# Lzcstan/DrugLAMP

Measured on AMD Instinct MI355X. Metric: drug-protein pairs/sec training step, higher is better.
Workload: dtype bf16; 1 GPU; DrugLAMP training step (cls step, epoch 1; fwd+bwd+grad all-reduce+AdamW), BindingDB-shaped synthetic pairs (512 drug nodes/tokens, 2304 protein tokens = 256 sites, pre-extracted 384-d/640-d LLM embeddings), global batch 256 = 256 per GPU x 1; per_gpu_batch=256, global_batch=256, parallelism=dp1, step_kind=cls, epoch=1, hip_graph=False, protein_seq_len=2304, distinct_batches=8, first_touch_steps=8, padding_rows=computed once, protein_cnn_rows=distinct rows, streams=independent branches on side HIP streams

## Files before the change

druglamp_amd/csrc/attention.hip:

```cpp
#include "tiles.cuh"

namespace {
using namespace dltile;

struct AttnP {
  const char *Q, *K, *V, *O, *dO;
  char *Out, *dQ, *dK, *dV;
  float *LSE, *Delta, *raw;
  int64_t q_ps, q_hs, q_rs, k_ps, k_hs, k_rs, v_ps, v_hs, v_rs, o_ps, o_hs, o_rs, o_ss;
  int64_t do_ps, do_hs, do_rs, do_ss, dq_ps, dq_hs, dq_rs, dk_ps, dk_hs, dk_rs, dv_ps, dv_hs, dv_rs;
  int P, H, S, shift, Lq, Lk;
  float scale;
  int algo;
  int tail_start;
  float tail_bias;
};

template <int QT, int NKT>
__device__ __forceinline__ void add_tail_bias_t(f32x4 (&s)[QT][NKT], int k0, int g, int tail_start, float tb) {
#pragma unroll
  for (int kt = 0; kt < NKT; ++kt)
#pragma unroll
    for (int r = 0; r < 4; ++r)
      if (k0 + kt * 16 + 4 * g + r >= tail_start) {
// ... 685 lines not shown
        sdo.store(dOs);
        if (threadIdx.x < QSB) {
          const int q = q0 + threadIdx.x;
          lse_s[threadIdx.x] = q < p.Lq ? p.LSE[statbase + q] * LOG2E : INFINITY;
          del_s[threadIdx.x] = q < p.Lq ? p.Delta[statbase + q] : 0.f;
        }
        __syncthreads();
        if (qb + 1 < nqb) {
          sq.load(Qb, p.q_rs, q0 + QSB, p.Lq);
          sdo.load(dOb, p.do_rs, q0 + QSB, p.Lq);
        }
      }
      const char* Qt = RES ? Qs + q0 * TL::RB : Qs;
      const char* dOt = RES ? dOs + q0 * TL::RB : dOs;
      const float* lse_t = RES ? lse_s + q0 : lse_s;
      const float* del_t = RES ? del_s + q0 : del_s;
      f32x4 s[KT][NQT], dp[KT][NQT];
#pragma unroll
      for (int qt = 0; qt < NQT; ++qt) {
#pragma unroll
        for (int kt = 0; kt < KT; ++kt) { s[kt][qt] = f32x4{0.f, 0.f, 0.f, 0.f}; dp[kt][qt] = f32x4{0.f, 0.f, 0.f, 0.f}; }
#pragma unroll
        for (int kf = 0; kf < NKF; ++kf) {
          const u32x4 qa = frag_kc<T, HD>(Qt, qt * 16, kf, il, g);
          const u32x4 da = frag_kc<T, HD>(dOt, qt * 16, kf, il, g);
#pragma unroll
          for (int kt = 0; kt < KT; ++kt) {
            s[kt][qt] = Mma<T>::mma(qa, kfr[kt][kf], s[kt][qt]);
            dp[kt][qt] = Mma<T>::mma(da, vfr[kt][kf], dp[kt][qt]);
          }
        }
        const f32x4 l4 = *reinterpret_cast<const f32x4*>(lse_t + qt * 16 + 4 * g);
        const f32x4 d4 = *reinterpret_cast<const f32x4*>(del_t + qt * 16 + 4 * g);
        if (has_tail) {
#pragma unroll
          for (int kt = 0; kt < KT; ++kt) s[kt][qt] += kbl[kt];
        }
#pragma unroll
        for (int kt = 0; kt < KT; ++kt)
#pragma unroll
          for (int r = 0; r < 4; ++r) {
            const float pv = fast_exp2(s[kt][qt][r] * c - l4[r]);
            s[kt][qt][r] = pv;
            dp[kt][qt][r] = pv * (dp[kt][qt][r] - d4[r]);
          }
      }
#pragma unroll
      for (int qp = 0; qp < NQP; ++qp) {
        u32x4 pb[KT], sb[KT];
#pragma unroll
        for (int kt = 0; kt < KT; ++kt) {
          pb[kt] = frag_from_acc<T>(&s[kt][qp * CT]);
          sb[kt] = frag_from_acc<T>(&dp[kt][qp * CT]);
        }
#pragma unroll
        for (int d = 0; d < NDT; ++d) {
          const u32x4 dota = frag_tr<T, HD>(dOt, qp * KF, d * 16, il, g);
          const u32x4 qta = frag_tr<T, HD>(Qt, qp * KF, d * 16, il, g);
#pragma unroll
          for (int kt = 0; kt < KT; ++kt) {
            dv[d][kt] = Mma<T>::mma(dota, pb[kt], dv[d][kt]);
            dk[d][kt] = Mma<T>::mma(qta, sb[kt], dk[d][kt]);
          }
        }
      }
      if constexpr (!RES) __syncthreads();
    }
  }
  T* dKb = reinterpret_cast<T*>(p.dK) + (int64_t)pa * p.dk_ps + (int64_t)h * p.dk_hs;
  T* dVb = reinterpret_cast<T*>(p.dV) + (int64_t)pa * p.dv_ps + (int64_t)h * p.dv_hs;
#pragma unroll
  for (int kt = 0; kt < KT; ++kt) {
    const int key = kw0 + kt * 16 + il;
    if (key < p.Lk) {
#pragma unroll
      for (int d = 0; d < NDT; ++d) {
        store4_fam<4, T>(dKb + (int64_t)key * p.dk_rs + d * 16 + 4 * g, dk[d][kt] * p.scale);
        store4_fam<4, T>(dVb + (int64_t)key * p.dv_rs + d * 16 + 4 * g, dv[d][kt]);
      }
    }
  }
}

template <typename T, int HD, int KT, bool TAILK = false>
__global__ __launch_bounds__(ATT_THREADS, 1) void attn_bwd_dkv_ring_kernel(const AttnP p) {
  using TL = ATile<T, HD>;
  constexpr int KF = Mma<T>::KF, NKF = HD / KF, NDT = HD / 16, CT = KF / 16;
  constexpr int QSB = 64, NQP = QSB / KF;
  constexpr int KVB = 4 * KT * 16;
  constexpr int TILE = QSB * TL::RB, STAGE = 2 * TILE;
  constexpr int NCH = QSB * TL::CPR / ATT_THREADS;
  static_assert(sizeof(T) == 2 && QSB * TL::CPR % ATT_THREADS == 0, "bf16 tiles, whole DMA instructions");
  __shared__ __attribute__((aligned(16))) char smem[2 * STAGE + 2 * 2 * QSB * sizeof(float)];
  const uint32_t smem_lds = (uint32_t)(size_t)(__attribute__((address_space(3))) char*)smem;
  float* stat_s = reinterpret_cast<float*>(smem + 2 * STAGE);
  const int tid = threadIdx.x, lane = tid & 63, wave = tid >> 6, il = lane & 15, g = lane >> 4;
  const int kb = blockIdx.x, h = blockIdx.y, pa = blockIdx.z;
  const T* Kb = reinterpret_cast<const T*>(p.K) + (int64_t)pa * p.k_ps + (int64_t)h * p.k_hs;
  const T* Vb = reinterpret_cast<const T*>(p.V) + (int64_t)pa * p.v_ps + (int64_t)h * p.v_hs;
  const int kw0 = kb * KVB + wave * KT * 16;
  const float c = p.scale * LOG2E;

  u32x4 kfr[KT][NKF], vfr[KT][NKF];
#pragma unroll
  for (int kt = 0; kt < KT; ++kt) {
    const int key = kw0 + kt * 16 + il;
    const bool ok = key < p.Lk;
#pragma unroll
    for (int kf = 0; kf < NKF; ++kf) {
      kfr[kt][kf] = frag_global<T>(Kb + (int64_t)key * p.k_rs, ok, kf, g);
      vfr[kt][kf] = frag_global<T>(Vb + (int64_t)key * p.v_rs, ok, kf, g);
    }
  }
  f32x4 dk[NDT][KT], dv[NDT][KT];
#pragma unroll
  for (int d = 0; d < NDT; ++d)
#pragma unroll
    for (int kt = 0; kt < KT; ++kt) { dk[d][kt] = f32x4{0.f, 0.f, 0.f, 0.f}; dv[d][kt] = f32x4{0.f, 0.f, 0.f, 0.f}; }
  const bool has_tail = TAILK && kw0 + KT * 16 > p.tail_start;
  float kbl[KT];
#pragma unroll
  for (int kt = 0; kt < KT; ++kt) kbl[kt] = (TAILK && kw0 + kt * 16 + il >= p.tail_start) ? p.tail_bias : 0.f;

  const int nqb = (p.Lq + QSB - 1) / QSB;
  for (int seg = 0; seg < p.S; ++seg) {
    const int qprob = seg == 0 ? pa : (pa + p.shift) % p.P;
    const T* Qb = reinterpret_cast<const T*>(p.Q) + (int64_t)qprob * p.q_ps + (int64_t)h * p.q_hs;
    const T* dOb = reinterpret_cast<const T*>(p.dO) + (int64_t)seg * p.do_ss + (int64_t)pa * p.do_ps + (int64_t)h * p.do_hs;
    const int64_t statbase = (((int64_t)seg * p.P + pa) * p.H + h) * p.Lq;
    auto issue = [&](int qb, int buf) {
      const char* zero = reinterpret_cast<const char*>(zero_page);
      const uint32_t sb = smem_lds + (uint32_t)buf * STAGE;
#pragma unroll
      for (int i = 0; i < NCH; ++i) {
        const int cc = tid + i * ATT_THREADS;
        const int row = cc / TL::CPR, ch = (cc % TL::CPR) ^ TL::swz(row);
        const int q = qb * QSB + row;
        const char* qs_ = q < p.Lq ? reinterpret_cast<const char*>(Qb + (int64_t)q * p.q_rs + ch * TL::EPC) : zero;
        const char* ds_ = q < p.Lq ? reinterpret_cast<const char*>(dOb + (int64_t)q * p.do_rs + ch * TL::EPC) : zero;
        const uint32_t off = __builtin_amdgcn_readfirstlane((uint32_t)((wave * 64 + i * ATT_THREADS) * 16));
        att_dma16(qs_, sb + off);
        att_dma16(ds_, sb + TILE + off);
      }
      if (tid < QSB) {
        const int q = qb * QSB + tid;
        stat_s[(buf * 2 + 0) * QSB + tid] = q < p.Lq ? p.LSE[statbase + q] * LOG2E : INFINITY;
        stat_s[(buf * 2 + 1) * QSB + tid] = q < p.Lq ? p.Delta[statbase + q] : 0.f;
      }
    };
    if (seg > 0) att_barrier();
    issue(0, 0);
    for (int qb = 0; qb < nqb; ++qb) {
      att_wait_all();
      att_barrier();
      if (qb + 1 < nqb) issue(qb + 1, (qb + 1) & 1);
      const char* Qt = smem + (qb & 1) * STAGE;
      const char* dOt = Qt + TILE;
      const float* lse_t = stat_s + ((qb & 1) * 2 + 0) * QSB;
      const float* del_t = stat_s + ((qb & 1) * 2 + 1) * QSB;
#pragma unroll
      for (int qp = 0; qp < NQP; ++qp) {
        f32x4 s[KT][CT], dp[KT][CT];
#pragma unroll
        for (int ci = 0; ci < CT; ++ci) {
          const int qt = qp * CT + ci;
#pragma unroll
          for (int kt = 0; kt < KT; ++kt) { s[kt][ci] = f32x4{0.f, 0.f, 0.f, 0.f}; dp[kt][ci] = f32x4{0.f, 0.f, 0.f, 0.f}; }
#pragma unroll
          for (int kf = 0; kf < NKF; ++kf) {
            const u32x4 qa = frag_kc<T, HD>(Qt, qt * 16, kf, il, g);
            const u32x4 da = frag_kc<T, HD>(dOt, qt * 16, kf, il, g);
#pragma unroll
            for (int kt = 0; kt < KT; ++kt) {
              s[kt][ci] = Mma<T>::mma(qa, kfr[kt][kf], s[kt][ci]);
              dp[kt][ci] = Mma<T>::mma(da, vfr[kt][kf], dp[kt][ci]);
            }
          }
          const f32x4 l4 = *reinterpret_cast<const f32x4*>(lse_t + qt * 16 + 4 * g);
          const f32x4 d4 = *reinterpret_cast<const f32x4*>(del_t + qt * 16 + 4 * g);
          if (has_tail) {
#pragma unroll
            for (int kt = 0; kt < KT; ++kt) s[kt][ci] += kbl[kt];
          }
#pragma unroll
          for (int kt = 0; kt < KT; ++kt)
#pragma unroll
            for (int r = 0; r < 4; ++r) {
              const float pv = fast_exp2(s[kt][ci][r] * c - l4[r]);
              s[kt][ci][r] = pv;
              dp[kt][ci][r] = pv * (dp[kt][ci][r] - d4[r]);
            }
        }
        u32x4 pb[KT], sb[KT];
#pragma unroll
        for (int kt = 0; kt < KT; ++kt) {
          pb[kt] = frag_from_acc<T>(&s[kt][0]);
          sb[kt] = frag_from_acc<T>(&dp[kt][0]);
        }
#pragma unroll
        for (int d = 0; d < NDT; ++d) {
          const u32x4 dota = frag_tr<T, HD>(dOt, qp * KF, d * 16, il, g);
          const u32x4 qta = frag_tr<T, HD>(Qt, qp * KF, d * 16, il, g);
#pragma unroll
          for (int kt = 0; kt < KT; ++kt) {
            dv[d][kt] = Mma<T>::mma(dota, pb[kt], dv[d][kt]);
            dk[d][kt] = Mma<T>::mma(qta, sb[kt], dk[d][kt]);
          }
        }
      }
    }
  }
  T* dKb = reinterpret_cast<T*>(p.dK) + (int64_t)pa * p.dk_ps + (int64_t)h * p.dk_hs;
  T* dVb = reinterpret_cast<T*>(p.dV) + (int64_t)pa * p.dv_ps + (int64_t)h * p.dv_hs;
#pragma unroll
  for (int kt = 0; kt < KT; ++kt) {
    const int key = kw0 + kt * 16 + il;
    if (key < p.Lk) {
#pragma unroll
      for (int d = 0; d < NDT; ++d) {
        store4_fam<4, T>(dKb + (int64_t)key * p.dk_rs + d * 16 + 4 * g, dk[d][kt] * p.scale);
        store4_fam<4, T>(dVb + (int64_t)key * p.dv_rs + d * 16 + 4 * g, dv[d][kt]);
      }
    }
  }
}

__device__ __forceinline__ int ds_swz(int key) { return (((key >> 2) & 1) << 1) | ((key >> 3) & 1); }
template <typename T, int HD>
__global__ __launch_bounds__(512, 1) void attn_bwd_fused_kernel(const AttnP p) {
  static_assert(sizeof(T) == 2 && HD == 64, "bf16, head_dim 64");
  using TL = ATile<T, HD>;
  constexpr int KF = Mma<T>::KF, NKF = HD / KF, NDT = HD / 16, KT = 2, NQT = 2, QBLK = 32, NT = 512, NST = 4;
  constexpr int TILE = QBLK * TL::RB;
  constexpr int STAGE = 3 * TILE;
  constexpr int IMG = 256 * TL::RB;
  constexpr int DSB = 256 * 64;
  __shared__ __attribute__((aligned(16))) char smem[NST * STAGE + 2 * IMG + 2 * DSB + NST * (64 + QBLK) * (int)sizeof(float)];
  char* ring = smem;
  char* Ks = smem + NST * STAGE;
  char* Vs = Ks + IMG;
  char* dSs = Vs + IMG;
  float* lse_s = reinterpret_cast<float*>(dSs + 2 * DSB);
  float* del_s = lse_s + NST * 64;
  const int tid = threadIdx.x, lane = tid & 63, il = lane & 15, g = lane >> 4;
  const int wave = __builtin_amdgcn_readfirstlane(tid >> 6);
  const int h = blockIdx.y;
  const int a0 = blockIdx.z;
  const int npass = p.S == 2 ? 4 : 1;
  const int kw0 = wave * KT * 16;
  const int qt_o = wave & 1, dt_o = wave >> 1;
  const float c = p.scale * LOG2E;
  const int nblk = (p.Lq + QBLK - 1) / QBLK;
  const int G = npass * nblk;
  const uint32_t smem_base = (uint32_t)(size_t)(__attribute__((address_space(3))) char*)smem;
  const char* zero = reinterpret_cast<const char*>(zero_page);

  const int nd = wave <= 4 ? 2 : 1;
  int pf_pass = 0, pf_blk = 0, pf_stage = 0;
  const T* pfA = nullptr;
  const T* pfO = nullptr;
  const float* pfL = nullptr;
  int64_t pfA_rs = 0;
  auto pf_setup = [&]() {
    const int pa = pf_pass < 2 ? a0 : a0 + p.shift;
    const int seg = pf_pass & 1;
    const int qprob = seg == 0 ? pa : (pa + p.shift) % p.P;
    if (wave < 4) { pfA = reinterpret_cast<const T*>(p.Q) + ((int64_t)qprob * p.q_ps + (int64_t)h * p.q_hs); pfA_rs = p.q_rs; }
    else { pfA = reinterpret_cast<const T*>(p.dO) + ((int64_t)seg * p.do_ss + (int64_t)pa * p.do_ps + (int64_t)h * p.do_hs); pfA_rs = p.do_rs; }
    pfO = reinterpret_cast<const T*>(p.O) + ((int64_t)seg * p.o_ss + (int64_t)pa * p.o_ps + (int64_t)h * p.o_hs);
    pfL = p.LSE + (((int64_t)seg * p.P + pa) * p.H + h) * p.Lq;
  };
  pf_setup();
  auto issue_next = [&]() {
    const uint32_t st = smem_base + (uint32_t)(pf_stage * STAGE);
    const int row = 8 * (wave & 3) + (lane >> 3), q = pf_blk * QBLK + row;
    const int ch = (lane & 7) ^ TL::swz(row);
    const bool ok = q < p.Lq;
    lds_dma16(ok ? reinterpret_cast<const char*>(pfA + (int64_t)q * pfA_rs + ch * TL::EPC) : zero,
              st + (uint32_t)((wave < 4 ? 0 : TILE) + (wave & 3) * 1024));
    if (wave < 4) {
      lds_dma16(ok ? reinterpret_cast<const char*>(pfO + (int64_t)q * p.o_rs + ch * TL::EPC) : zero, st + (uint32_t)(2 * TILE + wave * 1024));
    } else if (wave == 4) {
      const int ql = pf_blk * QBLK + (lane & 31);
      lds_dma4(pfL + (ql < p.Lq ? ql : p.Lq - 1), smem_base + (uint32_t)((char*)lse_s - smem) + (uint32_t)(pf_stage * 256));
    }
    pf_stage = (pf_stage + 1) & (NST - 1);
    if (++pf_blk == nblk) {
      pf_blk = 0;
      if (++pf_pass < npass) pf_setup();
    }
  };
  auto issue_kv = [&](int pa) {
    const T* Kb = reinterpret_cast<const T*>(p.K) + (int64_t)pa * p.k_ps + (int64_t)h * p.k_hs;
    const T* Vb = reinterpret_cast<const T*>(p.V) + (int64_t)pa * p.v_ps + (int64_t)h * p.v_hs;
#pragma unroll
    for (int i = 0; i < 4; ++i) {
      const int row = (i * 8 + wave) * 8 + (lane >> 3);
      const int ch = (lane & 7) ^ TL::swz(row);
      const bool ok = row < p.Lk;
      lds_dma16(ok ? reinterpret_cast<const char*>(Kb + (int64_t)row * p.k_rs + ch * TL::EPC) : zero,
                smem_base + (uint32_t)(Ks - smem) + (uint32_t)((i * 8 + wave) * 1024));
      lds_dma16(ok ? reinterpret_cast<const char*>(Vb + (int64_t)row * p.v_rs + ch * TL::EPC) : zero,
                smem_base + (uint32_t)(Vs - smem) + (uint32_t)((i * 8 + wave) * 1024));
    }
  };
// ... 69 lines not shown
            dp[kt] = Mma<T>::mma(da, vfr[kt][kf], dp[kt]);
          }
        }
        const f32x4 l4 = *reinterpret_cast<const f32x4*>(lse_t + qt * 16 + 4 * g) * LOG2E;
        const f32x4 d4 = *reinterpret_cast<const f32x4*>(del_t + qt * 16 + 4 * g);
#pragma unroll
        for (int kt = 0; kt < KT; ++kt) {
#pragma unroll
          for (int r = 0; r < 4; ++r) {
            const float pv = fast_exp2(s[kt][r] * c - l4[r]);
            s[kt][r] = pv;
            dp[kt][r] = pv * (dp[kt][r] - d4[r]);
          }
          pb[kt][2 * qt] = pack_bf16x2(s[kt][0], s[kt][1]);
          pb[kt][2 * qt + 1] = pack_bf16x2(s[kt][2], s[kt][3]);
          sb[kt][2 * qt] = pack_bf16x2(dp[kt][0], dp[kt][1]);
          sb[kt][2 * qt + 1] = pack_bf16x2(dp[kt][2], dp[kt][3]);
        }
      }
#pragma unroll
      for (int kt = 0; kt < KT; ++kt) {
        const int key = kw0 + kt * 16 + il, sw = ds_swz(key);
        *reinterpret_cast<u32x2*>(dSb + key * 64 + (((0 + (g >> 1)) ^ sw) << 4) + 8 * (g & 1)) = u32x2{sb[kt][0], sb[kt][1]};
        *reinterpret_cast<u32x2*>(dSb + key * 64 + (((2 + (g >> 1)) ^ sw) << 4) + 8 * (g & 1)) = u32x2{sb[kt][2], sb[kt][3]};
      }
#pragma unroll
      for (int d = 0; d < NDT; ++d) {
        const u32x4 dota = frag_tr<T, HD>(dOt, 0, d * 16, il, g);
        const u32x4 qta = frag_tr<T, HD>(Qt, 0, d * 16, il, g);
#pragma unroll
        for (int kt = 0; kt < KT; ++kt) {
          dv[d][kt] = Mma<T>::mma(dota, pb[kt], dv[d][kt]);
          dk[d][kt] = Mma<T>::mma(qta, sb[kt], dk[d][kt]);
        }
      }
      if (gb + 3 < G) {
        if (nd == 2) vm_wait<2>(); else vm_wait<1>();
      } else {
        vm_wait<0>();
      }
      __syncthreads();
      if (gb + 2 < G) form_delta((gb + 2) & (NST - 1));
      f32x4 dq = {0.f, 0.f, 0.f, 0.f};
#pragma unroll
      for (int cki = 0; cki < 8; ++cki) {
        const int r0 = cki * 32 + 4 * g + (il >> 2), sw = ds_swz(r0);
        const uint32_t off = (uint32_t)(r0 * 64 + (((2 * qt_o + ((il & 3) >> 1)) ^ sw) << 4) + (il & 1) * 8);
        const u32x2 lo = lds_read_tr16(dSb, off);
        const u32x2 hi = lds_read_tr16(dSb, off + 16 * 64);
        dq = Mma<T>::mma(ktr[cki], u32x4{lo[0], lo[1], hi[0], hi[1]}, dq);
      }
      if (add_share) asm volatile("s_waitcnt vmcnt(0)" : "+v"(prevw) :: "memory");
      if (qo < p.Lq) {
        f32x4 v = dq * p.scale;
        if (add_share) {
          v = v + f32x4{bf16lo(prevw[0]), bf16hi(prevw[0]), bf16lo(prevw[1]), bf16hi(prevw[1])};
          store4_fam<4, T>(dst, v);
        } else if (npass == 1) {
          store4_fam<4, T>(dst, v);
        } else {
          store4<T>(dst, v);
        }
      }
    }
    if (!new_kv || npass == 1) {
      T* dKb = reinterpret_cast<T*>(p.dK) + (int64_t)pa * p.dk_ps + (int64_t)h * p.dk_hs;
      T* dVb = reinterpret_cast<T*>(p.dV) + (int64_t)pa * p.dv_ps + (int64_t)h * p.dv_hs;
#pragma unroll
      for (int kt = 0; kt < KT; ++kt) {
        const int key = kw0 + kt * 16 + il;
        if (key < p.Lk) {
#pragma unroll
          for (int d = 0; d < NDT; ++d) {
            store4_fam<4, T>(dKb + (int64_t)key * p.dk_rs + d * 16 + 4 * g, dk[d][kt] * p.scale);
            store4_fam<4, T>(dVb + (int64_t)key * p.dv_rs + d * 16 + 4 * g, dv[d][kt]);
          }
        }
      }
    }
  }
}

template <typename T> constexpr int fwd_qt() { return sizeof(T) == 2 ? 2 : 1; }

int check_common(const char* who, int dtype, int head_dim, int nseg, int P, int H, int Lq, int Lk,
                 const int64_t* strides, int nstrides) {
  DL_CHECK_ARG(dtype == DL_F32 || dtype == DL_BF16, DL_ERR_ARG, "%s: bad dtype", who);
  DL_CHECK_ARG(head_dim == 64 || head_dim == 128, DL_ERR_UNSUPPORTED, "%s: head_dim %d not in {64,128}", who, head_dim);
  DL_CHECK_ARG(nseg == 1 || nseg == 2, DL_ERR_ARG, "%s: n_segments must be 1 or 2", who);
  DL_CHECK_ARG(P > 0 && H > 0 && Lq > 0 && Lk > 0 && P <= 65535 && H <= 65535, DL_ERR_SHAPE, "%s: bad sizes", who);
  const int epc = 16 / (int)dl_dtype_size(dtype);
  for (int i = 0; i < nstrides; ++i)
    DL_CHECK_ARG(strides[i] % epc == 0, DL_ERR_ALIGN, "%s: stride #%d (%ld) not a multiple of %d elements", who,
                 i, (long)strides[i], epc);
  return DL_OK;
}

template <typename T, int HD>
int launch_fwd(const AttnP& p, hipStream_t s) {
  if constexpr (sizeof(T) == 2) {
    if (HD == 64 && p.Lk <= 256 && p.algo != DL_ATTN_ALGO_STREAM && p.tail_start >= p.Lk) {
      constexpr int NW = HD == 64 ? 4 : 8;
      hipLaunchKernelGGL((attn_fwd_res_kernel<T, HD, 2, NW>), dim3((uint32_t)p.H, (uint32_t)p.P), dim3(64 * NW), 0, s, p);
      return DL_OK;
    }
  }
  constexpr int QT = fwd_qt<T>();
  constexpr int QB = 4 * QT * 16;
  dim3 grid((uint32_t)(p.S * ((p.Lq + QB - 1) / QB)), (uint32_t)p.H, (uint32_t)p.P);
  if constexpr (sizeof(T) == 2 && HD == 64) {
    if (!p.raw && p.Lq <= 64) {
      const dim3 g1((uint32_t)(p.S * ((p.Lq + 63) / 64)), (uint32_t)p.H, (uint32_t)p.P);
      hipLaunchKernelGGL((attn_fwd_kernel<T, HD, 1, 64, 4>), g1, dim3(ATT_THREADS), 0, s, p);
      return DL_OK;
    }
    if (!p.raw && p.Lk >= 1024) {
      hipLaunchKernelGGL((attn_fwd_kernel<T, HD, QT, 128>), grid, dim3(ATT_THREADS), 0, s, p);
      return DL_OK;
    }
  }
  hipLaunchKernelGGL((attn_fwd_kernel<T, HD, QT>), grid, dim3(ATT_THREADS), 0, s, p);
  return DL_OK;
}

template <typename T, int HD>
int launch_bwd(const AttnP& p, hipStream_t s) {
  constexpr int QT = fwd_qt<T>();
  constexpr int QB = 4 * QT * 16;
  constexpr int KT = sizeof(T) == 2 ? 2 : 1;
  constexpr int KVB = 4 * KT * 16;
  const dim3 gq((uint32_t)((p.Lq + QB - 1) / QB), (uint32_t)p.H, (uint32_t)p.P);
  const dim3 gk((uint32_t)((p.Lk + KVB - 1) / KVB), (uint32_t)p.H, (uint32_t)p.P);
  if constexpr (sizeof(T) == 2 && HD == 64) {
    const int64_t nwg = (int64_t)p.H * (p.S == 2 ? p.shift : p.P);
    if (p.Lk <= 256 && (p.S == 1 || 2 * p.shift == p.P) && p.tail_start >= p.Lk &&
        (p.algo == DL_ATTN_ALGO_ONE_PASS || (p.algo == DL_ATTN_ALGO_AUTO && nwg >= 256))) {
      const dim3 gf(1u, (uint32_t)p.H, (uint32_t)(p.S == 2 ? p.shift : p.P));
      hipLaunchKernelGGL((attn_bwd_fused_kernel<T, HD>), gf, dim3(512), 0, s, p);
      return DL_OK;
    }
    if (p.Lk <= 256 && p.Lq <= 256 && p.algo != DL_ATTN_ALGO_STREAM && p.tail_start >= p.Lk) {
      hipLaunchKernelGGL((attn_bwd_dq_kernel<T, HD, QT, true>), gq, dim3(ATT_THREADS), 0, s, p);
      hipLaunchKernelGGL((attn_bwd_dkv_kernel<T, HD, KT, true>), gk, dim3(ATT_THREADS), 0, s, p);
      return DL_OK;
    }
  }
  if constexpr (sizeof(T) != 2) {
    const int64_t rows = (int64_t)p.S * p.P * p.H * p.Lq;
    hipLaunchKernelGGL((attn_delta_kernel<T, HD>), dim3((uint32_t)((rows + 15) / 16)), dim3(256), 0, s, p);
  }
  if constexpr (sizeof(T) == 2 && HD == 128) {
    if (p.tail_start < p.Lk) {
      hipLaunchKernelGGL((attn_bwd_dq_ring_kernel<T, HD, QT, true>), gq, dim3(ATT_THREADS), 0, s, p);
      hipLaunchKernelGGL((attn_bwd_dkv_ring_kernel<T, HD, KT, true>), gk, dim3(ATT_THREADS), 0, s, p);
    } else {
      hipLaunchKernelGGL((attn_bwd_dq_ring_kernel<T, HD, QT>), gq, dim3(ATT_THREADS), 0, s, p);
      hipLaunchKernelGGL((attn_bwd_dkv_ring_kernel<T, HD, KT>), gk, dim3(ATT_THREADS), 0, s, p);
    }
  } else {
    hipLaunchKernelGGL((attn_bwd_dq_kernel<T, HD, QT, false>), gq, dim3(ATT_THREADS), 0, s, p);
    hipLaunchKernelGGL((attn_bwd_dkv_kernel<T, HD, KT, false>), gk, dim3(ATT_THREADS), 0, s, p);
  }
  return DL_OK;
}

template <typename Args>
int fill_common(const char* who, const Args* a, AttnP& p) {
  p.Q = (const char*)a->Q; p.K = (const char*)a->K; p.V = (const char*)a->V;
  p.q_ps = a->q_ps; p.q_hs = a->q_hs; p.q_rs = a->q_rs; p.k_ps = a->k_ps; p.k_hs = a->k_hs; p.k_rs = a->k_rs;
  p.v_ps = a->v_ps; p.v_hs = a->v_hs; p.v_rs = a->v_rs; p.o_ps = a->o_ps; p.o_hs = a->o_hs; p.o_rs = a->o_rs;
  p.o_ss = a->o_ss;
  p.P = a->n_problems; p.H = a->n_heads; p.S = a->n_segments; p.shift = a->partner_shift;
  p.Lq = a->Lq; p.Lk = a->Lk; p.scale = a->scale; p.algo = a->algo;
  DL_CHECK_ARG(a->key_tail_rows >= 0 && a->key_tail_rows <= a->Lk && (a->key_tail_rows == 0 || (a->key_tail_weight >= 1.f && a->scale > 0.f)),
               DL_ERR_ARG, "%s: key_tail_rows in [0, Lk], key_tail_weight >= 1", who);
  DL_CHECK_ARG(a->key_tail_rows == 0 || a->n_segments == 1, DL_ERR_UNSUPPORTED, "%s: key multiplicities with one segment only", who);
  p.tail_start = a->Lk - a->key_tail_rows;
  p.tail_bias = a->key_tail_rows ? logf(a->key_tail_weight) / a->scale : 0.f;
  return DL_OK;
}

}

extern "C" int dl_attn_fwd(const dl_attn_fwd_args* a, dl_stream stream) {
  hipStream_t s = (hipStream_t)stream;
  DL_CHECK_ARG(a && a->Q && a->K && a->V && a->O, DL_ERR_ARG, "dl_attn_fwd: null pointer");
  const int64_t st[] = {a->q_ps, a->q_hs, a->q_rs, a->k_ps, a->k_hs, a->k_rs, a->v_ps, a->v_hs,
                        a->v_rs, a->o_ps, a->o_hs, a->o_rs, a->o_ss};
  int rc = check_common("dl_attn_fwd", a->dtype, a->head_dim, a->n_segments, a->n_problems, a->n_heads,
                        a->Lq, a->Lk, st, 13);
  if (rc != DL_OK) return rc;
  DL_CHECK_ARG(a->n_segments == 1 || (a->partner_shift >= 0 && a->partner_shift < a->n_problems),
               DL_ERR_ARG, "dl_attn_fwd: bad partner_shift");
  AttnP p = {};
  rc = fill_common("dl_attn_fwd", a, p);
  if (rc != DL_OK) return rc;
  p.Out = (char*)a->O; p.LSE = a->LSE; p.raw = a->raw_logits;
  dl_prof_before(1, s);
  if (a->dtype == DL_BF16) rc = a->head_dim == 64 ? launch_fwd<bf16_t, 64>(p, s) : launch_fwd<bf16_t, 128>(p, s);
  else rc = a->head_dim == 64 ? launch_fwd<float, 64>(p, s) : launch_fwd<float, 128>(p, s);
  DL_CHECK_LAUNCH("dl_attn_fwd");
  const double nq = (double)a->n_segments * a->n_problems * a->n_heads * a->Lq;
  const int es = (int)dl_dtype_size(a->dtype);
  dl_prof_after(1, s, 4.0 * nq * a->Lk * a->head_dim,
                (2.0 * nq + 2.0 * a->n_problems * a->n_heads * a->Lk) * a->head_dim * es);
  return rc;
}

extern "C" int dl_attn_bwd(const dl_attn_bwd_args* a, dl_stream stream) {
  hipStream_t s = (hipStream_t)stream;
  DL_CHECK_ARG(a && a->Q && a->K && a->V && a->O && a->dO && a->LSE && a->Delta && a->dQ && a->dK && a->dV,
               DL_ERR_ARG, "dl_attn_bwd: null pointer");
  const int64_t st[] = {a->q_ps, a->q_hs, a->q_rs, a->k_ps, a->k_hs, a->k_rs, a->v_ps, a->v_hs, a->v_rs,
                        a->o_ps, a->o_hs, a->o_rs, a->o_ss, a->do_ps, a->do_hs, a->do_rs, a->do_ss,
                        a->dq_ps, a->dq_hs, a->dq_rs, a->dk_ps, a->dk_hs, a->dk_rs, a->dv_ps, a->dv_hs, a->dv_rs};
  int rc = check_common("dl_attn_bwd", a->dtype, a->head_dim, a->n_segments, a->n_problems, a->n_heads,
                        a->Lq, a->Lk, st, 26);
  if (rc != DL_OK) return rc;
  DL_CHECK_ARG(a->n_segments == 1 || (a->partner_shift >= 0 && a->partner_shift < a->n_problems),
               DL_ERR_ARG, "dl_attn_bwd: bad partner_shift");
  AttnP p = {};
  rc = fill_common("dl_attn_bwd", a, p);
  if (rc != DL_OK) return rc;
  p.O = (const char*)a->O; p.dO = (const char*)a->dO; p.LSE = const_cast<float*>(a->LSE); p.Delta = a->Delta;
  p.dQ = (char*)a->dQ; p.dK = (char*)a->dK; p.dV = (char*)a->dV;
  p.do_ps = a->do_ps; p.do_hs = a->do_hs; p.do_rs = a->do_rs; p.do_ss = a->do_ss;
  p.dq_ps = a->dq_ps; p.dq_hs = a->dq_hs; p.dq_rs = a->dq_rs; p.dk_ps = a->dk_ps; p.dk_hs = a->dk_hs;
  p.dk_rs = a->dk_rs; p.dv_ps = a->dv_ps; p.dv_hs = a->dv_hs; p.dv_rs = a->dv_rs;
  dl_prof_before(2, s);
  if (a->dtype == DL_BF16) rc = a->head_dim == 64 ? launch_bwd<bf16_t, 64>(p, s) : launch_bwd<bf16_t, 128>(p, s);
  else rc = a->head_dim == 64 ? launch_bwd<float, 64>(p, s) : launch_bwd<float, 128>(p, s);
  DL_CHECK_LAUNCH("dl_attn_bwd");
  const double nq = (double)a->n_segments * a->n_problems * a->n_heads * a->Lq;
  const int es = (int)dl_dtype_size(a->dtype);
  dl_prof_after(2, s, 10.0 * nq * a->Lk * a->head_dim,
                (4.0 * nq + 4.0 * a->n_problems * a->n_heads * a->Lk) * a->head_dim * es);
  return rc;
}
```

druglamp_amd/ops.py:

```python
from __future__ import annotations

import contextlib
import ctypes as C
import math
import os
from typing import Optional

import torch

from . import _lib
from ._lib import (DL_BF16, DL_F32, AttnBwdArgs, AttnFwdArgs, AttnProbsArgs, GemmArgs, PgcaPairsArgs, PgcaPairsAttrArgs, PgcaPairsProbsArgs,
                   PgcaPairsProfileArgs, PgcaPairsRaggedArgs, PgcaPairsRaggedAttrArgs, PgcaPairsRaggedProbsArgs, PgcaPairsRaggedProfileArgs,
                   check)

_DT = {torch.float32: DL_F32, torch.bfloat16: DL_BF16}


def _dt(t: torch.Tensor) -> int:
    try:
        return _DT[t.dtype]
    except KeyError:
        raise TypeError("druglamp_amd: unsupported dtype %s (float32 / bfloat16 only)" % t.dtype)


# ... 244 lines not shown
                      ws.data_ptr(), ws.numel(), _stream()), "dl_colsum")
    return out


def layernorm_fwd(x2d, gamma, beta, eps):
    _need_gpu(x2d, gamma, beta)
    L = _lib.lib()
    M, D = x2d.shape
    y = torch.empty_like(x2d)
    mean = torch.empty(M, dtype=torch.float32, device=x2d.device)
    rstd = torch.empty(M, dtype=torch.float32, device=x2d.device)
    check(L.dl_layernorm_fwd(x2d.data_ptr(), x2d.stride(0), gamma.data_ptr(), beta.data_ptr(), y.data_ptr(),
                             y.stride(0), mean.data_ptr(), rstd.data_ptr(), M, D, float(eps), _dt(x2d), _stream()),
          "dl_layernorm_fwd")
    return y, mean, rstd


def layernorm_bwd(dy2d, x2d, mean, rstd, gamma, dres=None, need_param_grads=True, out=None, dy_share=1):
    L = _lib.lib()
    M, D = x2d.shape
    if dy2d.shape[0] * dy_share != M:
        raise ValueError("layernorm_bwd: dy has %d rows, x %d, dy_share %d" % (dy2d.shape[0], M, dy_share))
    dx = torch.empty_like(x2d) if out is None else out
    dgamma = dbeta = None
    if need_param_grads:
        gb = torch.empty((2, D), dtype=torch.float32, device=x2d.device)
        dgamma, dbeta = gb[0], gb[1]
    nbytes = L.dl_layernorm_bwd_workspace_bytes(M, D)
    item = None
    if _pending is not None and need_param_grads:
        ws = torch.empty(nbytes, dtype=torch.uint8, device=x2d.device)
        item = _lib.ReduceItem()
    else:
        ws = _ws.get(nbytes, x2d.device)
    check(L.dl_layernorm_bwd(dy2d.data_ptr(), dy2d.stride(0), int(dy_share), x2d.data_ptr(), x2d.stride(0), mean.data_ptr(),
                             rstd.data_ptr(), gamma.data_ptr(), _ptr(dres), 0 if dres is None else dres.stride(0),
                             dx.data_ptr(), dx.stride(0), _ptr(dgamma), _ptr(dbeta), 0, M, D, _dt(x2d),
                             ws.data_ptr(), ws.numel(), None if item is None else C.pointer(item), _stream()), "dl_layernorm_bwd")
    if item is not None and item.kind != 0:
        _pending.append((item, ws, gb, None))
    return dx, dgamma, dbeta


def cast(src: torch.Tensor, dtype: torch.dtype) -> torch.Tensor:
    if src.dtype == dtype:
        return src
    _need_gpu(src)
    src = src.contiguous()
    dst = torch.empty(src.shape, dtype=dtype, device=src.device)
    check(_lib.lib().dl_cast(src.data_ptr(), _dt(src), dst.data_ptr(), _DT[dtype], src.numel(), _stream()), "dl_cast")
    return dst


def attn_fwd(q, k, v, *, n_problems, n_heads, n_segments, partner_shift, Lq, Lk, head_dim, scale,
             q_strides, k_strides, v_strides, out, o_strides, o_ss, need_lse=True, raw_logits=None, algo=0, key_tail=None):
    _need_gpu(q, k, v, out)
    a = AttnFwdArgs()
    a.Q, a.K, a.V, a.O = q.data_ptr(), k.data_ptr(), v.data_ptr(), out.data_ptr()
    lse = None
    if need_lse:
        lse = torch.empty((n_segments, n_problems, n_heads, Lq), dtype=torch.float32, device=q.device)
    a.LSE = _ptr(lse)
    a.raw_logits = _ptr(raw_logits)
    a.q_ps, a.q_hs, a.q_rs = q_strides
    a.k_ps, a.k_hs, a.k_rs = k_strides
    a.v_ps, a.v_hs, a.v_rs = v_strides
    a.o_ps, a.o_hs, a.o_rs = o_strides
    a.o_ss = o_ss
    a.n_problems, a.n_heads, a.n_segments, a.partner_shift = n_problems, n_heads, n_segments, partner_shift
    a.Lq, a.Lk, a.head_dim, a.dtype = Lq, Lk, head_dim, _dt(q)
    a.scale = float(scale)
    a.algo = algo
    if key_tail is not None:
        a.key_tail_rows, a.key_tail_weight = int(key_tail[0]), float(key_tail[1])
    check(_lib.lib().dl_attn_fwd(C.byref(a), _stream()), "dl_attn_fwd")
    return lse


_ATTN_BWD_ALGO = int(os.environ.get("DL_ATTN_BWD_ALGO", "0"))


def attn_bwd(q, k, v, o, do, lse, *, n_problems, n_heads, n_segments, partner_shift, Lq, Lk, head_dim, scale,
             q_strides, k_strides, v_strides, o_strides, o_ss, do_strides, do_ss, dq, dq_strides, dk, dk_strides,
             dv, dv_strides, algo=0, key_tail=None):
    _need_gpu(q, k, v, o, do)
    a = AttnBwdArgs()
    delta = torch.empty_like(lse)
    a.Q, a.K, a.V, a.O, a.dO = q.data_ptr(), k.data_ptr(), v.data_ptr(), o.data_ptr(), do.data_ptr()
    a.LSE, a.Delta = lse.data_ptr(), delta.data_ptr()
    a.dQ, a.dK, a.dV = dq.data_ptr(), dk.data_ptr(), dv.data_ptr()
    a.q_ps, a.q_hs, a.q_rs = q_strides
    a.k_ps, a.k_hs, a.k_rs = k_strides
    a.v_ps, a.v_hs, a.v_rs = v_strides
    a.o_ps, a.o_hs, a.o_rs = o_strides
    a.o_ss = o_ss
    a.do_ps, a.do_hs, a.do_rs = do_strides
    a.do_ss = do_ss
    a.dq_ps, a.dq_hs, a.dq_rs = dq_strides
    a.dk_ps, a.dk_hs, a.dk_rs = dk_strides
    a.dv_ps, a.dv_hs, a.dv_rs = dv_strides
    a.n_problems, a.n_heads, a.n_segments, a.partner_shift = n_problems, n_heads, n_segments, partner_shift
    a.Lq, a.Lk, a.head_dim, a.dtype = Lq, Lk, head_dim, _dt(q)
    a.scale = float(scale)
    a.algo = algo if algo else _ATTN_BWD_ALGO
    if key_tail is not None:
        a.key_tail_rows, a.key_tail_weight = int(key_tail[0]), float(key_tail[1])
    check(_lib.lib().dl_attn_bwd(C.byref(a), _stream()), "dl_attn_bwd")


def attn_probs(q, k, *, n_problems, n_heads, n_segments, partner_shift, Lq, Lk, head_dim, scale, q_strides, k_strides,
               lse=None, head_mean=False, key_tail=None, expand_tail=False, out=None, out_ld=None):
    _need_gpu(q, k, lse, out)
    a = AttnProbsArgs()
    a.Q, a.K, a.LSE = q.data_ptr(), k.data_ptr(), _ptr(lse)
    a.q_ps, a.q_hs, a.q_rs = q_strides
    a.k_ps, a.k_hs, a.k_rs = k_strides
    a.n_problems, a.n_heads, a.n_segments, a.partner_shift = n_problems, n_heads, n_segments, partner_shift
    a.Lq, a.Lk, a.head_dim, a.dtype = Lq, Lk, head_dim, _dt(q)
    a.scale = float(scale)
    a.head_mean, a.expand_tail = int(bool(head_mean)), int(bool(expand_tail))
    cols = Lk
    if key_tail is not None:
        a.key_tail_rows, a.key_tail_weight = int(key_tail[0]), float(key_tail[1])
        if expand_tail:
            cols = Lk - int(key_tail[0]) + int(key_tail[0]) * int(key_tail[1])
    if lse is not None and (lse.dtype != torch.float32 or not lse.is_contiguous() or lse.numel() != n_segments * n_problems * n_heads * Lq):
        raise ValueError("attn_probs: lse must be a contiguous float32 tensor of (n_segments, n_problems, n_heads, Lq)")
    if out is None:
        shape = (n_segments, n_problems, Lq, cols) if head_mean else (n_segments, n_problems, n_heads, Lq, cols)
        out = torch.empty(shape, dtype=torch.float32, device=q.device)
        out_ld = cols
    else:
        rows = n_segments * n_problems * (1 if head_mean else n_heads) * Lq
        if out.dtype != torch.float32 or out_ld is None or not out.is_contiguous() or out.device != q.device:
            raise ValueError("attn_probs: out must be a contiguous float32 tensor on q's device and come with its row pitch out_ld")
        if out_ld < cols or out.numel() < (rows - 1) * int(out_ld) + cols:
            raise ValueError("attn_probs: out holds %d elements, %d rows of %d columns at pitch %d need %d"
                             % (out.numel(), rows, cols, out_ld, (rows - 1) * int(out_ld) + cols))
    a.out, a.out_ld = out.data_ptr(), int(out_ld)
    L = _lib.lib()
    if lse is None:
        ws = _ws.get(L.dl_attn_probs_workspace_bytes(C.byref(a)), q.device)
        a.workspace, a.workspace_bytes = ws.data_ptr(), ws.numel()
    check(L.dl_attn_probs(C.byref(a), _stream()), "dl_attn_probs")
    return out


def _check_pair_operands(who, q, store, store_name, store_dims, q_index, kv_index):
    if (q.dim() != 3 or store.dim() != len(store_dims) + 1 or q.shape[2] != 128 or store.shape[-1] != 256 or q.stride(2) != 1
            or store.stride(-1) != 1):
        raise ValueError("%s: q must be (n_q, Lq, 128) and %s (%s, 256) with contiguous columns" % (who, store_name, ", ".join(store_dims)))
    if store.dtype != q.dtype:
        raise ValueError("%s: q is %s, %s is %s" % (who, q.dtype, store_name, store.dtype))
    for t in (q_index, kv_index):
        if t.dtype != torch.int32 or t.dim() != 1 or not t.is_contiguous() or t.numel() != q_index.numel():
            raise ValueError("%s: q_index / kv_index must be contiguous int32 vectors of one length" % who)


def _fill_pair_head(a, q, store, q_index, kv_index, scale):
    a.Q, a.K = q.data_ptr(), store.data_ptr()
    a.q_index, a.kv_index, a.flags = q_index.data_ptr(), kv_index.data_ptr(), guard_flags(q.device).data_ptr()
    a.q_es, a.q_rs = q.stride(0), q.stride(1)
    a.k_rs = store.stride(-2)
    a.n_pairs, (a.n_q, a.Lq, a.head_dim), a.dtype = q_index.numel(), q.shape, _dt(q)
    a.scale = float(scale)


def _check_cols(who, cols):
    cols = int(cols)
    if cols < 1:
# ... 974 lines not shown
```

Before: 20660 pairs/s.

## Make attention dK/dV backward kernel persistent with a 4-stage DMA pipeline

Turns the dK/dV ring backward kernel into a persistent kernel. The grid is capped at 256 blocks, and each block walks a contiguous run of (kb, h, pa) work items. K/V tiles and Q/dO tiles, plus LSE/Delta stats, stream through a single 4-stage LDS ring using async DMA and vmcnt waits. This is meant to hide load latency across work items and remove per-block launch and prologue cost. It also double-buffers LDS fragment reads with sched_group_barrier hints to interleave them with MFMAs. It adds a lot of pipeline-accounting complexity, and the larger LDS footprint can reduce occupancy. The Python side gains an optional delta buffer argument.

```diff
diff --git a/druglamp_amd/csrc/attention.hip b/druglamp_amd/csrc/attention.hip
--- a/druglamp_amd/csrc/attention.hip
+++ b/druglamp_amd/csrc/attention.hip
@@ -791,145 +791,235 @@
   }
 }
 
+__device__ __forceinline__ void item_run(int nitems, int& first, int& count) {
+  const int G = (int)gridDim.x, b = (int)blockIdx.x;
+  const int base = nitems / G, rem = nitems % G;
+  first = b * base + (b < rem ? b : rem);
+  count = base + (b < rem ? 1 : 0);
+}
+__device__ __attribute__((aligned(16))) const uint32_t inf_page[4] = {0x7f800000u, 0x7f800000u, 0x7f800000u, 0x7f800000u};
+
 template <typename T, int HD, int KT, bool TAILK = false>
 __global__ __launch_bounds__(ATT_THREADS, 1) void attn_bwd_dkv_ring_kernel(const AttnP p) {
   using TL = ATile<T, HD>;
   constexpr int KF = Mma<T>::KF, NKF = HD / KF, NDT = HD / 16, CT = KF / 16;
   constexpr int QSB = 64, NQP = QSB / KF;
-  constexpr int KVB = 4 * KT * 16;
+  constexpr int KVB = 4 * KT * 16, KVE = KVB / QSB;
   constexpr int TILE = QSB * TL::RB, STAGE = 2 * TILE;
+  constexpr int NST = 4, AHEAD = NST - 1;
   constexpr int NCH = QSB * TL::CPR / ATT_THREADS;
+  constexpr int PER = 2 * NCH + 1;
   static_assert(sizeof(T) == 2 && QSB * TL::CPR % ATT_THREADS == 0, "bf16 tiles, whole DMA instructions");
-  __shared__ __attribute__((aligned(16))) char smem[2 * STAGE + 2 * 2 * QSB * sizeof(float)];
+  static_assert(KVB % QSB == 0 && QSB % (KT * 16) == 0 && AHEAD == 3 && 2 * PER < 64, "entry layout, vmcnt immediates");
+  __shared__ __attribute__((aligned(16))) char smem[NST * STAGE + NST * 2 * QSB * sizeof(float)];
   const uint32_t smem_lds = (uint32_t)(size_t)(__attribute__((address_space(3))) char*)smem;
-  float* stat_s = reinterpret_cast<float*>(smem + 2 * STAGE);
-  const int tid = threadIdx.x, lane = tid & 63, wave = tid >> 6, il = lane & 15, g = lane >> 4;
-  const int kb = blockIdx.x, h = blockIdx.y, pa = blockIdx.z;
-  const T* Kb = reinterpret_cast<const T*>(p.K) + (int64_t)pa * p.k_ps + (int64_t)h * p.k_hs;
-  const T* Vb = reinterpret_cast<const T*>(p.V) + (int64_t)pa * p.v_ps + (int64_t)h * p.v_hs;
-  const int kw0 = kb * KVB + wave * KT * 16;
+  const float* stat_s = reinterpret_cast<const float*>(smem + NST * STAGE);
+  const int tid = threadIdx.x, lane = tid & 63, il = lane & 15, g = lane >> 4;
+  const int wave = __builtin_amdgcn_readfirstlane(tid >> 6);
   const float c = p.scale * LOG2E;
-
+  const int nkb = (p.Lk + KVB - 1) / KVB, nqb = (p.Lq + QSB - 1) / QSB;
+  const int nq = p.S * nqb, ne = KVE + nq;
+  int first, count;
+  item_run(nkb * p.H * p.P, first, count);
+  if (count == 0) return;
+  const int64_t G = (int64_t)count * ne;
+  const char* zero = reinterpret_cast<const char*>(zero_page);
+
+  int pf_kb = first % nkb, pf_h = (first / nkb) % p.H, pf_pa = first / (nkb * p.H), pf_e = 0, pf_stage = 0;
+  auto issue_next = [&]() {
+    const T *A, *B;
+    int64_t a_rs, b_rs;
+    int row0, lim;
+    const float* stat = nullptr;
+    if (pf_e < KVE) {
+      A = reinterpret_cast<const T*>(p.K) + (int64_t)pf_pa * p.k_ps + (int64_t)pf_h * p.k_hs;
+      B = reinterpret_cast<const T*>(p.V) + (int64_t)pf_pa * p.v_ps + (int64_t)pf_h * p.v_hs;
+      a_rs = p.k_rs; b_rs = p.v_rs; row0 = pf_kb * KVB + pf_e * QSB; lim = p.Lk;
+    } else {
+      const int seg = pf_e - KVE >= nqb ? 1 : 0, qb = pf_e - KVE - seg * nqb;
+      const int qprob = seg == 0 ? pf_pa : (pf_pa + p.shift) % p.P;
+      A = reinterpret_cast<const T*>(p.Q) + (int64_t)qprob * p.q_ps + (int64_t)pf_h * p.q_hs;
+      B = reinterpret_cast<const T*>(p.dO) + (int64_t)seg * p.do_ss + (int64_t)pf_pa * p.do_ps + (int64_t)pf_h * p.do_hs;
+      a_rs = p.q_rs; b_rs = p.do_rs; row0 = qb * QSB; lim = p.Lq;
+      stat = ((wave & 1) ? p.Delta : p.LSE) + (((int64_t)seg * p.P + pf_pa) * p.H + pf_h) * p.Lq;
+    }
+    const uint32_t sb = smem_lds + (uint32_t)(pf_stage * STAGE);
+    int tl = tid;
+    asm volatile("" : "+v"(tl));
+#pragma unroll
+    for (int i = 0; i < NCH; ++i) {
+      const int cc = tl + i * ATT_THREADS;
+      const int row = cc / TL::CPR, ch = (cc % TL::CPR) ^ TL::swz(row);
+      const int r = row0 + row;
+      const char* as_ = r < lim ? reinterpret_cast<const char*>(A + (int64_t)r * a_rs + ch * TL::EPC) : zero;
+      const char* bs_ = r < lim ? reinterpret_cast<const char*>(B + (int64_t)r * b_rs + ch * TL::EPC) : zero;
+      const uint32_t off = (uint32_t)((wave * 64 + i * ATT_THREADS) * 16);
+      lds_dma16(as_, sb + off);
+      lds_dma16(bs_, sb + TILE + off);
+    }
+    {
+      const int q = row0 + (tl & 63);
+      const void* src = (stat && q < lim) ? reinterpret_cast<const void*>(stat + q)
+                                          : reinterpret_cast<const void*>((wave & 1) ? zero_page : inf_page);
+      lds_dma4(src, smem_lds + (uint32_t)(NST * STAGE + (pf_stage * 2 + (wave & 1)) * QSB * (int)sizeof(float)));
+    }
+    pf_stage = (pf_stage + 1) & (NST - 1);
+    if (++pf_e == ne) {
+      pf_e = 0;
+      if (++pf_kb == nkb) {
+        pf_kb = 0;
+        if (++pf_h == p.H) { pf_h = 0; ++pf_pa; }
+      }
+    }
+  };
+  int64_t gb = 0;
+  auto begin_entry = [&]() {
+    att_barrier();
+    if (gb + AHEAD < G) issue_next();
+  };
+  auto end_entry = [&]() {
+    const int64_t newer = G - gb - 2;
+    if (newer >= 2) vm_wait<2 * PER>();
+    else if (newer == 1) vm_wait<PER>();
+    else vm_wait<0>();
+    ++gb;
+  };
   u32x4 kfr[KT][NKF], vfr[KT][NKF];
-#pragma unroll
-  for (int kt = 0; kt < KT; ++kt) {
-    const int key = kw0 + kt * 16 + il;
-    const bool ok = key < p.Lk;
-#pragma unroll
-    for (int kf = 0; kf < NKF; ++kf) {
-      kfr[kt][kf] = frag_global<T>(Kb + (int64_t)key * p.k_rs, ok, kf, g);
-      vfr[kt][kf] = frag_global<T>(Vb + (int64_t)key * p.v_rs, ok, kf, g);
-    }
-  }
-  f32x4 dk[NDT][KT], dv[NDT][KT];
-#pragma unroll
-  for (int d = 0; d < NDT; ++d)
-#pragma unroll
-    for (int kt = 0; kt < KT; ++kt) { dk[d][kt] = f32x4{0.f, 0.f, 0.f, 0.f}; dv[d][kt] = f32x4{0.f, 0.f, 0.f, 0.f}; }
-  const bool has_tail = TAILK && kw0 + KT * 16 > p.tail_start;
-  float kbl[KT];
-#pragma unroll
-  for (int kt = 0; kt < KT; ++kt) kbl[kt] = (TAILK && kw0 + kt * 16 + il >= p.tail_start) ? p.tail_bias : 0.f;
-
-  const int nqb = (p.Lq + QSB - 1) / QSB;
-  for (int seg = 0; seg < p.S; ++seg) {
-    const int qprob = seg == 0 ? pa : (pa + p.shift) % p.P;
-    const T* Qb = reinterpret_cast<const T*>(p.Q) + (int64_t)qprob * p.q_ps + (int64_t)h * p.q_hs;
-    const T* dOb = reinterpret_cast<const T*>(p.dO) + (int64_t)seg * p.do_ss + (int64_t)pa * p.do_ps + (int64_t)h * p.do_hs;
-    const int64_t statbase = (((int64_t)seg * p.P + pa) * p.H + h) * p.Lq;
-    auto issue = [&](int qb, int buf) {
-      const char* zero = reinterpret_cast<const char*>(zero_page);
-      const uint32_t sb = smem_lds + (uint32_t)buf * STAGE;
-#pragma unroll
-      for (int i = 0; i < NCH; ++i) {
-        const int cc = tid + i * ATT_THREADS;
-        const int row = cc / TL::CPR, ch = (cc % TL::CPR) ^ TL::swz(row);
-        const int q = qb * QSB + row;
-        const char* qs_ = q < p.Lq ? reinterpret_cast<const char*>(Qb + (int64_t)q * p.q_rs + ch * TL::EPC) : zero;
-        const char* ds_ = q < p.Lq ? reinterpret_cast<const char*>(dOb + (int64_t)q * p.do_rs + ch * TL::EPC) : zero;
-        const uint32_t off = __builtin_amdgcn_readfirstlane((uint32_t)((wave * 64 + i * ATT_THREADS) * 16));
-        att_dma16(qs_, sb + off);
-        att_dma16(ds_, sb + TILE + off);
-      }
-      if (tid < QSB) {
-        const int q = qb * QSB + tid;
-        stat_s[(buf * 2 + 0) * QSB + tid] = q < p.Lq ? p.LSE[statbase + q] * LOG2E : INFINITY;
-        stat_s[(buf * 2 + 1) * QSB + tid] = q < p.Lq ? p.Delta[statbase + q] : 0.f;
-      }
-    };
-    if (seg > 0) att_barrier();
-    issue(0, 0);
-    for (int qb = 0; qb < nqb; ++qb) {
-      att_wait_all();
-      att_barrier();
-      if (qb + 1 < nqb) issue(qb + 1, (qb + 1) & 1);
-      const char* Qt = smem + (qb & 1) * STAGE;
-      const char* dOt = Qt + TILE;
-      const float* lse_t = stat_s + ((qb & 1) * 2 + 0) * QSB;
-      const float* del_t = stat_s + ((qb & 1) * 2 + 1) * QSB;
-#pragma unroll
-      for (int qp = 0; qp < NQP; ++qp) {
-        f32x4 s[KT][CT], dp[KT][CT];
-#pragma unroll
-        for (int ci = 0; ci < CT; ++ci) {
-          const int qt = qp * CT + ci;
-#pragma unroll
-          for (int kt = 0; kt < KT; ++kt) { s[kt][ci] = f32x4{0.f, 0.f, 0.f, 0.f}; dp[kt][ci] = f32x4{0.f, 0.f, 0.f, 0.f}; }
+  auto load_kv = [&]() {
+#pragma unroll
+    for (int e = 0; e < KVE; ++e) {
+      begin_entry();
+      const char* Kt = smem + (int)(gb & (NST - 1)) * STAGE;
+      const char* Vt = Kt + TILE;
+      if (wave * KT * 16 / QSB == e) {
+        const int r0 = wave * KT * 16 - e * QSB;
+#pragma unroll
+        for (int kt = 0; kt < KT; ++kt)
 #pragma unroll
           for (int kf = 0; kf < NKF; ++kf) {
-            const u32x4 qa = frag_kc<T, HD>(Qt, qt * 16, kf, il, g);
-            const u32x4 da = frag_kc<T, HD>(dOt, qt * 16, kf, il, g);
+            kfr[kt][kf] = frag_kc<T, HD>(Kt, r0 + kt * 16, kf, il, g);
+            vfr[kt][kf] = frag_kc<T, HD>(Vt, r0 + kt * 16, kf, il, g);
+          }
+      }
+      end_entry();
+    }
+  };
+
+  for (int t = 0; t < AHEAD; ++t) issue_next();
+  vm_wait<2 * PER>();
+  load_kv();
+  int kb = first % nkb, h = (first / nkb) % p.H, pa = first / (nkb * p.H);
+  for (int it = 0; it < count; ++it) {
+    const int kw0 = kb * KVB + wave * KT * 16;
+    const bool live = kw0 < p.Lk;
+    f32x4 dk[NDT][KT], dv[NDT][KT];
+#pragma unroll
+    for (int d = 0; d < NDT; ++d)
+#pragma unroll
+      for (int kt = 0; kt < KT; ++kt) { dk[d][kt] = f32x4{0.f, 0.f, 0.f, 0.f}; dv[d][kt] = f32x4{0.f, 0.f, 0.f, 0.f}; }
+    const bool has_tail = TAILK && kw0 + KT * 16 > p.tail_start;
+    float kbl[KT];
+#pragma unroll
+    for (int kt = 0; kt < KT; ++kt) kbl[kt] = (TAILK && kw0 + kt * 16 + il >= p.tail_start) ? p.tail_bias : 0.f;
+
+    if (!live) {
+      for (int e = 0; e < nq; ++e) { begin_entry(); end_entry(); }
+    } else {
+      for (int e = 0; e < nq; ++e) {
+        begin_entry();
+        const int sg = (int)(gb & (NST - 1));
+        const char* Qt = smem + sg * STAGE;
+        const char* dOt = Qt + TILE;
+        const float* lse_t = stat_s + (sg * 2 + 0) * QSB;
+        const float* del_t = stat_s + (sg * 2 + 1) * QSB;
+#pragma unroll
+        for (int qp = 0; qp < NQP; ++qp) {
+          f32x4 s[KT][CT], dp[KT][CT];
+          u32x4 qa[2], da[2];
+          qa[0] = frag_kc<T, HD>(Qt, qp * CT * 16, 0, il, g);
+          da[0] = frag_kc<T, HD>(dOt, qp * CT * 16, 0, il, g);
+          __builtin_amdgcn_sched_group_barrier(0x100, 2, 0);
+#pragma unroll
+          for (int ci = 0; ci < CT; ++ci) {
+            const int qt = qp * CT + ci;
+#pragma unroll
+            for (int kt = 0; kt < KT; ++kt) { s[kt][ci] = f32x4{0.f, 0.f, 0.f, 0.f}; dp[kt][ci] = f32x4{0.f, 0.f, 0.f, 0.f}; }
+#pragma unroll
+            for (int kf = 0; kf < NKF; ++kf) {
+              const int n = ci * NKF + kf;
+              if (n + 1 < CT * NKF) {
+                qa[(n + 1) & 1] = frag_kc<T, HD>(Qt, (qp * CT + (n + 1) / NKF) * 16, (n + 1) % NKF, il, g);
+                da[(n + 1) & 1] = frag_kc<T, HD>(dOt, (qp * CT + (n + 1) / NKF) * 16, (n + 1) % NKF, il, g);
+                __builtin_amdgcn_sched_group_barrier(0x100, 2, 0);
+              }
+#pragma unroll
+              for (int kt = 0; kt < KT; ++kt) {
+                s[kt][ci] = Mma<T>::mma(qa[n & 1], kfr[kt][kf], s[kt][ci]);
+                dp[kt][ci] = Mma<T>::mma(da[n & 1], vfr[kt][kf], dp[kt][ci]);
+              }
+              __builtin_amdgcn_sched_group_barrier(0x008, 2 * KT, 0);
+            }
+            f32x4 l4 = *reinterpret_cast<const f32x4*>(lse_t + qt * 16 + 4 * g) * LOG2E;
+            asm volatile("" : "+v"(l4));
+            const f32x4 d4 = *reinterpret_cast<const f32x4*>(del_t + qt * 16 + 4 * g);
+            if (has_tail) {
+#pragma unroll
+              for (int kt = 0; kt < KT; ++kt) s[kt][ci] += kbl[kt];
+            }
+#pragma unroll
+            for (int kt = 0; kt < KT; ++kt)
+#pragma unroll
+              for (int r = 0; r < 4; ++r) {
+                const float pv = fast_exp2(s[kt][ci][r] * c - l4[r]);
+                s[kt][ci][r] = pv;
+                dp[kt][ci][r] = pv * (dp[kt][ci][r] - d4[r]);
+              }
+          }
+          u32x4 pb[KT], sb[KT];
+#pragma unroll
+          for (int kt = 0; kt < KT; ++kt) {
+            pb[kt] = frag_from_acc<T>(&s[kt][0]);
+            sb[kt] = frag_from_acc<T>(&dp[kt][0]);
+          }
+          u32x4 dota[2], qta[2];
+          dota[0] = frag_tr<T, HD>(dOt, qp * KF, 0, il, g);
+          qta[0] = frag_tr<T, HD>(Qt, qp * KF, 0, il, g);
+          __builtin_amdgcn_sched_group_barrier(0x100, 4, 0);
+#pragma unroll
+          for (int d = 0; d < NDT; ++d) {
+            if (d + 1 < NDT) {
+              dota[(d + 1) & 1] = frag_tr<T, HD>(dOt, qp * KF, (d + 1) * 16, il, g);
+              qta[(d + 1) & 1] = frag_tr<T, HD>(Qt, qp * KF, (d + 1) * 16, il, g);
+              __builtin_amdgcn_sched_group_barrier(0x100, 4, 0);
+            }
 #pragma unroll
             for (int kt = 0; kt < KT; ++kt) {
-              s[kt][ci] = Mma<T>::mma(qa, kfr[kt][kf], s[kt][ci]);
-              dp[kt][ci] = Mma<T>::mma(da, vfr[kt][kf], dp[kt][ci]);
+              dv[d][kt] = Mma<T>::mma(dota[d & 1], pb[kt], dv[d][kt]);
+              dk[d][kt] = Mma<T>::mma(qta[d & 1], sb[kt], dk[d][kt]);
             }
-          }
-          const f32x4 l4 = *reinterpret_cast<const f32x4*>(lse_t + qt * 16 + 4 * g);
-          const f32x4 d4 = *reinterpret_cast<const f32x4*>(del_t + qt * 16 + 4 * g);
-          if (has_tail) {
-#pragma unroll
-            for (int kt = 0; kt < KT; ++kt) s[kt][ci] += kbl[kt];
-          }
-#pragma unroll
-          for (int kt = 0; kt < KT; ++kt)
-#pragma unroll
-            for (int r = 0; r < 4; ++r) {
-              const float pv = fast_exp2(s[kt][ci][r] * c - l4[r]);
-              s[kt][ci][r] = pv;
-              dp[kt][ci][r] = pv * (dp[kt][ci][r] - d4[r]);
-            }
-        }
-        u32x4 pb[KT], sb[KT];
-#pragma unroll
-        for (int kt = 0; kt < KT; ++kt) {
-          pb[kt] = frag_from_acc<T>(&s[kt][0]);
-          sb[kt] = frag_from_acc<T>(&dp[kt][0]);
-        }
+            __builtin_amdgcn_sched_group_barrier(0x008, 2 * KT, 0);
+          }
+        }
+        end_entry();
+      }
+    }
+    if (it + 1 < count) load_kv();
+    T* dKb = reinterpret_cast<T*>(p.dK) + (int64_t)pa * p.dk_ps + (int64_t)h * p.dk_hs;
+    T* dVb = reinterpret_cast<T*>(p.dV) + (int64_t)pa * p.dv_ps + (int64_t)h * p.dv_hs;
+#pragma unroll
+    for (int kt = 0; kt < KT; ++kt) {
+      const int key = kw0 + kt * 16 + il;
+      if (key < p.Lk) {
 #pragma unroll
         for (int d = 0; d < NDT; ++d) {
-          const u32x4 dota = frag_tr<T, HD>(dOt, qp * KF, d * 16, il, g);
-          const u32x4 qta = frag_tr<T, HD>(Qt, qp * KF, d * 16, il, g);
-#pragma unroll
-          for (int kt = 0; kt < KT; ++kt) {
-            dv[d][kt] = Mma<T>::mma(dota, pb[kt], dv[d][kt]);
-            dk[d][kt] = Mma<T>::mma(qta, sb[kt], dk[d][kt]);
-          }
-        }
-      }
-    }
-  }
-  T* dKb = reinterpret_cast<T*>(p.dK) + (int64_t)pa * p.dk_ps + (int64_t)h * p.dk_hs;
-  T* dVb = reinterpret_cast<T*>(p.dV) + (int64_t)pa * p.dv_ps + (int64_t)h * p.dv_hs;
-#pragma unroll
-  for (int kt = 0; kt < KT; ++kt) {
-    const int key = kw0 + kt * 16 + il;
-    if (key < p.Lk) {
-#pragma unroll
-      for (int d = 0; d < NDT; ++d) {
-        store4_fam<4, T>(dKb + (int64_t)key * p.dk_rs + d * 16 + 4 * g, dk[d][kt] * p.scale);
-        store4_fam<4, T>(dVb + (int64_t)key * p.dv_rs + d * 16 + 4 * g, dv[d][kt]);
-      }
+          store4_fam<4, T>(dKb + (int64_t)key * p.dk_rs + d * 16 + 4 * g, dk[d][kt] * p.scale);
+          store4_fam<4, T>(dVb + (int64_t)key * p.dv_rs + d * 16 + 4 * g, dv[d][kt]);
+        }
+      }
+    }
+    if (++kb == nkb) {
+      kb = 0;
+      if (++h == p.H) { h = 0; ++pa; }
     }
   }
 }
@@ -1165,6 +1255,7 @@
 }
 
 template <typename T> constexpr int fwd_qt() { return sizeof(T) == 2 ? 2 : 1; }
+constexpr int ATT_CUS = 256;
 
 int check_common(const char* who, int dtype, int head_dim, int nseg, int P, int H, int Lq, int Lk,
                  const int64_t* strides, int nstrides) {
@@ -1233,12 +1324,15 @@
     hipLaunchKernelGGL((attn_delta_kernel<T, HD>), dim3((uint32_t)((rows + 15) / 16)), dim3(256), 0, s, p);
   }
   if constexpr (sizeof(T) == 2 && HD == 128) {
+    const int64_t kitems = (int64_t)gk.x * p.H * p.P;
+    DL_CHECK_ARG(kitems <= INT32_MAX, DL_ERR_SHAPE, "dl_attn_bwd: too many work items");
+    const dim3 gki((uint32_t)(p.algo == DL_ATTN_ALGO_STREAM ? kitems : std::min<int64_t>(kitems, ATT_CUS)));
     if (p.tail_start < p.Lk) {
       hipLaunchKernelGGL((attn_bwd_dq_ring_kernel<T, HD, QT, true>), gq, dim3(ATT_THREADS), 0, s, p);
-      hipLaunchKernelGGL((attn_bwd_dkv_ring_kernel<T, HD, KT, true>), gk, dim3(ATT_THREADS), 0, s, p);
+      hipLaunchKernelGGL((attn_bwd_dkv_ring_kernel<T, HD, KT, true>), gki, dim3(ATT_THREADS), 0, s, p);
     } else {
       hipLaunchKernelGGL((attn_bwd_dq_ring_kernel<T, HD, QT>), gq, dim3(ATT_THREADS), 0, s, p);
-      hipLaunchKernelGGL((attn_bwd_dkv_ring_kernel<T, HD, KT>), gk, dim3(ATT_THREADS), 0, s, p);
+      hipLaunchKernelGGL((attn_bwd_dkv_ring_kernel<T, HD, KT>), gki, dim3(ATT_THREADS), 0, s, p);
     }
   } else {
     hipLaunchKernelGGL((attn_bwd_dq_kernel<T, HD, QT, false>), gq, dim3(ATT_THREADS), 0, s, p);
diff --git a/druglamp_amd/ops.py b/druglamp_amd/ops.py
--- a/druglamp_amd/ops.py
+++ b/druglamp_amd/ops.py
@@ -350,10 +350,11 @@
 
 def attn_bwd(q, k, v, o, do, lse, *, n_problems, n_heads, n_segments, partner_shift, Lq, Lk, head_dim, scale,
              q_strides, k_strides, v_strides, o_strides, o_ss, do_strides, do_ss, dq, dq_strides, dk, dk_strides,
-             dv, dv_strides, algo=0, key_tail=None):
+             dv, dv_strides, algo=0, key_tail=None, delta=None):
     _need_gpu(q, k, v, o, do)
     a = AttnBwdArgs()
-    delta = torch.empty_like(lse)
+    if delta is None:
+        delta = torch.empty_like(lse)
     a.Q, a.K, a.V, a.O, a.dO = q.data_ptr(), k.data_ptr(), v.data_ptr(), o.data_ptr(), do.data_ptr()
     a.LSE, a.Delta = lse.data_ptr(), delta.data_ptr()
     a.dQ, a.dK, a.dV = dq.data_ptr(), dk.data_ptr(), dv.data_ptr()
```

Measured after the change: 18870 pairs/s. 8.6% lower.
